# ruanyyyyyyy/point-cloud-process

Hardware: AMD Instinct MI355X
Metric: correspondence-pairs/sec + ms/ICP-iter, 120k-pt KITTI pair (higher is better)
Workload: dtype f64; 1 GPU; point-to-point ICP iteration, 120000 x 120000 KITTI-shaped synthetic scan pair per GPU (BASELINE configs[1]); exact 1-NN via grid; nn=grid, pairs_per_gpu=1, points_src=120000, points_tgt=120000

## Files before the change

### point-cloud-process_amd/csrc/pcr_grid_search.hip

```cpp
#include <atomic>
#include <chrono>
#include <cmath>
#include <cstdlib>
#include <cstring>
#include "pcr_descent.h"
#include "pcr_icp_step.h"

constexpr unsigned int HARD_SCAN_T = 192;
constexpr int HARD_STACK = 160;
constexpr long long ID_NONE = 0x7fffffffffffffffll;
constexpr int H_NLIST = 32;
constexpr int H_CSTRIDE = 32;
__host__ __device__ static inline unsigned int hard_list_cap(long long nq) {
    const long long halves = (nq + 15) / 16;
    return (unsigned int)(((halves + H_NLIST - 1) / H_NLIST) * 16 + 64);
}

template <int G>
__device__ static inline void group_best(double& bd2, long long& bid, unsigned int& bpos) {
#pragma unroll
    for (int off = G / 2; off > 0; off >>= 1) {
        const double od2 = __shfl_xor(bd2, off, 64);
        const long long oid = __shfl_xor(bid, off, 64);
        const unsigned int opos = __shfl_xor(bpos, off, 64);
// ... 757 lines not shown
                win[k] = readlane_f64(bw[k], wl);
        }
    }
}

__global__ void __launch_bounds__(256)
grid_hard_kernel(pcr_grid_view gv, const work_item* __restrict__ list, const unsigned int* __restrict__ count_p, long long nq, double max_d2, int gated,
                 unsigned int* __restrict__ res_pos, double* __restrict__ res_d2, unsigned long long* __restrict__ dbg,
                 const pcr_icp_dev_state* __restrict__ st) {
    __shared__ hard_lds s_lds[4];
    if (st && st->stop) return;
    const int lane = threadIdx.x & 63, wave = threadIdx.x >> 6;
    hard_lds* L = &s_lds[wave];
    unsigned int l_cnt = lane < H_NLIST ? count_p[H_CSTRIDE * lane] : 0u;
    unsigned int l_inc = l_cnt;
#pragma unroll
    for (int off = 1; off < H_NLIST; off <<= 1) {
        const unsigned int o = __shfl_up(l_inc, off, 64);
        if (lane >= off) l_inc += o;
    }
    const unsigned int count = __shfl(l_inc, H_NLIST - 1, 64);
    const unsigned int l_exc = l_inc - l_cnt;
    const unsigned int l_cap = hard_list_cap(nq);
    for (unsigned int w = blockIdx.x * 4 + wave; w < count; w += gridDim.x * 4) {
        const int hl = (int)__ffsll((long long)__ballot(lane < H_NLIST && l_exc <= w && w < l_exc + l_cnt)) - 1;
        const work_item it = list[(size_t)hl * l_cap + (w - __shfl(l_exc, hl, 64))];
        const unsigned long long h_t0 = dbg ? __builtin_amdgcn_s_memtime() : 0;
        unsigned int h_steps = 0, h_pts = 0;
        int s_level0 = 0;
        double bd2;
        long long bid;
        unsigned int bpos;
        hard_search(gv, L, lane, it.ax, it.ay, it.az, gated ? fmin(it.best_d2, max_d2) : it.best_d2, it.best_pos != POS_NONE, bd2, bid, bpos, h_steps,
                    h_pts, s_level0);
        if (lane == 0) {
            res_pos[it.qi] = bpos;
            if (res_d2) res_d2[it.qi] = bd2;
            if (dbg && w < 60000) {
                dbg[(1 << 17) + w * 4 + 0] = __builtin_amdgcn_s_memtime() - h_t0;
                dbg[(1 << 17) + w * 4 + 1] = ((unsigned long long)h_steps << 32);
                dbg[(1 << 17) + w * 4 + 2] = h_pts;
                dbg[(1 << 17) + w * 4 + 3] = (unsigned long long)(it.best_pos != POS_NONE) | ((unsigned long long)(s_level0 + 1) << 8);
            }
        }
    }
}

constexpr int ACC_SETS = 32;
constexpr double GATE_KAPPA = 1.25;
constexpr int PASS_GROUPS = 32;
constexpr int PASS_SYNC_STRIDE = 32;
constexpr int PASS_SYNC_WORDS = PASS_SYNC_STRIDE * (PASS_GROUPS + 1);
constexpr unsigned long long ITEM_NONE = ~0ull;
constexpr unsigned int POISON_HI = 0xfffffffeu;
__device__ static inline unsigned long long item_poison(unsigned int pass_id) { return ((unsigned long long)POISON_HI << 32) | pass_id; }
#ifndef PCR_PASS_SPIN_LIMIT
#define PCR_PASS_SPIN_LIMIT (1u << 21)
#endif
constexpr unsigned int PASS_SPIN_LIMIT = PCR_PASS_SPIN_LIMIT;
constexpr int Q_BITS = 22;
constexpr unsigned long long Q_MASK = (1ull << Q_BITS) - 1ull;
constexpr long long PASS_MAX_NQ = 1ll << 26;
struct pass_args {
    unsigned long long* items;
    unsigned long long* sync;
    unsigned int cap;
    unsigned long long* acc;
    wt_xyz* prev_xyz;
    unsigned long long* gate_lb;
    unsigned long long* gate_est;
    double scale, inv_scale;
    double lin, inv_lin;
    pcr_icp_dev_state* st;
    pcr_icp_loop_args la;
    unsigned int* tile_cost;
    unsigned int pass_id;
    unsigned long long* host_block;
    unsigned int notify;
    unsigned int* plog;
};
constexpr int PASS_LOG_WORDS = 3 * PCR_ICP_MAX_LOG + 8;
constexpr size_t HOST_LOG_OFF = (sizeof(pcr_icp_dev_state) + 63) & ~(size_t)63;
constexpr size_t HOST_FLAG_OFF = 8192 - 8;
static_assert(HOST_LOG_OFF + 4 * PASS_LOG_WORDS <= HOST_FLAG_OFF, "state + pass log + flag fit the landing block");
__host__ __device__ static inline unsigned int pass_item_cap(long long nq) {
    const long long tiles = (nq + WT_Q - 1) / WT_Q + 4;
    return (unsigned int)(((tiles + PASS_GROUPS - 1) / PASS_GROUPS) * (WT_Q + 1));
}

__device__ static inline long long to_fixed(double v, double scale) {
    constexpr double BIG = 6755399441055744.0;
    return __double_as_longlong(__builtin_fma(v, scale, BIG)) - __double_as_longlong(BIG);
}

__device__ static inline bool mom_is_linear(int k) { return k >= 1 && k <= 6; }
__device__ static inline void acc_fixed_add(unsigned long long* __restrict__ acc, unsigned int set, int lane, double mk, double scale, double lin) {
    if (lane < PCR_NMOM - 1 && mk != 0.0)
        atomicAdd(acc + (size_t)(set % ACC_SETS) * PCR_NMOM + lane, (unsigned long long)to_fixed(mk, mom_is_linear(lane) ? scale * lin : scale));
}

__device__ static inline void acc_fixed_add_ll(unsigned long long* __restrict__ acc, unsigned int set, int lane, long long v) {
    if (lane < PCR_NMOM - 1 && v != 0) atomicAdd(acc + (size_t)(set % ACC_SETS) * PCR_NMOM + lane, (unsigned long long)v);
}

__device__ static inline unsigned long long ld_dev(const unsigned long long* p) {
    return __hip_atomic_load(p, __ATOMIC_RELAXED, __HIP_MEMORY_SCOPE_AGENT);
}
__device__ static inline void st_dev(unsigned long long* p, unsigned long long v) {
    __hip_atomic_store(p, v, __ATOMIC_RELAXED, __HIP_MEMORY_SCOPE_AGENT);
}

constexpr int LAND_WORD = 18, LAND_ROOT = 24;
constexpr int LAND_PUB_SHIFT = 20, LAND_IN_SHIFT = 42;
constexpr unsigned long long LAND_TILE_MASK = (1ull << LAND_PUB_SHIFT) - 1ull;
constexpr unsigned long long TICKET_FIN = 1ull << 63;
static_assert(LAND_IN_SHIFT - LAND_PUB_SHIFT == Q_BITS && LAND_IN_SHIFT + Q_BITS == 64, "landed word: 20 + 22 + 22 bits");
__device__ __forceinline__ static bool land_complete(unsigned long long now, unsigned int g_tiles) {
    return (unsigned int)(now & LAND_TILE_MASK) == g_tiles && ((now >> LAND_PUB_SHIFT) & Q_MASK) == (now >> LAND_IN_SHIFT);
}
__device__ __forceinline__ static bool land_report_item(unsigned long long* sync, int lane, unsigned int qi, unsigned int n_waves, unsigned int n_groups) {
    asm volatile("s_waitcnt vmcnt(0)" ::: "memory");
    int fin = 0;
    if (lane == 0) {
        const unsigned int pg = (qi / WT_Q) % PASS_GROUPS;
        const unsigned long long now = __hip_atomic_fetch_add(sync + (size_t)PASS_SYNC_STRIDE * pg + LAND_WORD, 1ull << LAND_IN_SHIFT, __ATOMIC_RELAXED, __HIP_MEMORY_SCOPE_AGENT) +
                                       (1ull << LAND_IN_SHIFT);
        if (land_complete(now, n_waves / PASS_GROUPS + (pg < n_waves % PASS_GROUPS ? 1u : 0u)))
            fin = __hip_atomic_fetch_add(sync + (size_t)PASS_SYNC_STRIDE * PASS_GROUPS + LAND_ROOT, 1ull, __ATOMIC_RELAXED, __HIP_MEMORY_SCOPE_AGENT) == (unsigned long long)(n_groups - 1u) ? 1 : 0;
    }
    return __builtin_amdgcn_readfirstlane(fin) != 0;
}
__device__ __forceinline__ static int ticket_root(unsigned long long* root, unsigned long long tg_old, bool left_by_poison, bool failed, bool fin, unsigned int n_groups,
                                                  int& fin_seen) {
    const bool g_clean = ((tg_old >> 32) & 0xffffull) != 0 || left_by_poison;
    const bool g_failed = ((tg_old >> 48) & 0x7fffull) != 0 || failed;
    const bool g_fin = (tg_old & TICKET_FIN) != 0 || fin;
    const unsigned long long tr_old = __hip_atomic_fetch_add(root, 1ull | (g_clean ? 1ull << 32 : 0ull) | (g_failed ? 1ull << 48 : 0ull) | (g_fin ? TICKET_FIN : 0ull), __ATOMIC_RELAXED,
                                                             __HIP_MEMORY_SCOPE_AGENT);
    if ((unsigned int)tr_old != n_groups - 1u) return 0;
    fin_seen = ((tr_old & TICKET_FIN) != 0 || g_fin) ? 1 : 0;
    int last = ((unsigned int)((tr_old >> 32) & 0xffffull) + (g_clean ? 1u : 0u) == n_groups) ? 1 : 2;
    if (((tr_old >> 48) & 0x7fffull) != 0 || g_failed) last = 3;
    return last;
}

union pass_lds {
    wtile_lds t;
    hard_lds h;
    double xch[WT_Q * (PCR_NMOM - 1)];
    long long xll[WT_Q * (PCR_NMOM - 1)];
};

__device__ __forceinline__ static unsigned int pass_serve_item(const pcr_grid_view& gv, pass_lds* L, const int lane, const unsigned long long w, const double max_d2,
                                                       const pass_args& A, unsigned int* __restrict__ res_pos, unsigned long long* __restrict__ dbg,
                                                       const unsigned int dbg_slot, const unsigned long long t_start) {
    const unsigned int w_lo = (unsigned int)w, w_hi = (unsigned int)(w >> 32);
    const double ax = __hiloint2double(__builtin_amdgcn_readlane((int)w_hi, 0), __builtin_amdgcn_readlane((int)w_lo, 0));
    const double ay = __hiloint2double(__builtin_amdgcn_readlane((int)w_hi, 1), __builtin_amdgcn_readlane((int)w_lo, 1));
    const double az = __hiloint2double(__builtin_amdgcn_readlane((int)w_hi, 2), __builtin_amdgcn_readlane((int)w_lo, 2));
    const unsigned int qi = (unsigned int)__builtin_amdgcn_readlane((int)w_lo, 3);
    const float cand_b2 = __uint_as_float((unsigned int)__builtin_amdgcn_readlane((int)w_hi, 3));
    const unsigned long long h_t0 = dbg ? __builtin_amdgcn_s_memtime() : 0;
    unsigned int h_steps = 0, h_pts = 0;
    int s_level0 = 0;
    double bd2;
    long long bid;
    unsigned int bpos;
    const bool have_cand = cand_b2 < INFINITY;
    const bool wide = A.gate_est != nullptr && !have_cand;
    const double wide_d2 = max_d2 * (GATE_KAPPA * GATE_KAPPA);
    bool inside = false;
    double win[3];
    hard_search(gv, &L->h, lane, ax, ay, az, have_cand ? fmin((double)cand_b2, max_d2) : (wide ? wide_d2 : max_d2), have_cand, bd2, bid, bpos, h_steps, h_pts, s_level0, win);
    wave_sync();
    if (bpos != POS_NONE) {
        if (lane == 0) {
            pcr_pt b;
            b.x = win[0]; b.y = win[1]; b.z = win[2]; b.id = 0;
            double m[PCR_NMOM];
#pragma unroll
            for (int k = 0; k < PCR_NMOM; ++k) m[k] = 0.0;
            moments_add(m, gv.origin, ax, ay, az, b, max_d2, 1);
            inside = m[0] != 0.0;
            if (!wide || inside) A.prev_xyz[qi] = wt_xyz{b.x, b.y, b.z};
#pragma unroll
            for (int k = 0; k < PCR_NMOM - 1; ++k) L->xch[k] = m[k];
        }
// ... 208 lines not shown
    const unsigned int g = tile % PASS_GROUPS;
    const unsigned int g_tiles = n_waves / PASS_GROUPS + (g < n_waves % PASS_GROUPS ? 1u : 0u);
    unsigned long long* const g_q = A.sync + (size_t)PASS_SYNC_STRIDE * g;
    unsigned long long* const g_started = g_q + 16;
    unsigned long long* const g_ticket = g_q + 17;
    unsigned long long* const items = A.items + (size_t)g * A.cap * 4;
    if (lane == 0) __hip_atomic_fetch_add(g_started, 1ull, __ATOMIC_RELAXED, __HIP_MEMORY_SCOPE_AGENT);
    const unsigned int n_groups = n_waves < (unsigned int)PASS_GROUPS ? n_waves : (unsigned int)PASS_GROUPS;
    wt_state S;
    wtile_search(*gvp, &L->t, tile, lane, P, q, nq, x, 1, 1, max_d2, 1, pcap, res_pos, nullptr, dbg, use_prev ? A.prev_xyz : nullptr, S, inline_queue ? A.sync + 16 : nullptr,
                 (unsigned int)PASS_SYNC_STRIDE, n_groups, n_waves, use_prev ? A.gate_lb : nullptr, A.gate_est, A.pass_id);
    tile_record_cost(S, lane, A.tile_cost, tile);
    if (dbg) rt_tile = __builtin_amdgcn_s_memrealtime();
    tile_nb nb;
    tile_neighbour(gv.pts, S, P, lane, nb);
    bool all_started = false;
    if (inline_queue) {
        all_started = S.probe != 0;
        if (!all_started) {
            unsigned long long sv = 0;
            if (lane < (int)n_groups) sv = ld_dev(A.sync + (size_t)PASS_SYNC_STRIDE * lane + 16);
            const bool ok = lane < (int)n_groups && (unsigned int)sv == n_waves / PASS_GROUPS + ((unsigned int)lane < n_waves % PASS_GROUPS ? 1u : 0u);
            all_started = __ballot(ok) == (n_groups >= 64 ? ~0ull : (1ull << n_groups) - 1ull);
        }
    }
    const bool unres = S.open && lane < WT_Q;
    const unsigned long long um = __ballot(unres);
    unsigned int mine = 0;
    bool have_claim = false;
    unsigned long long own = 0;
    unsigned long long* const root = A.sync + (size_t)PASS_SYNC_STRIDE * PASS_GROUPS;
    {
        unsigned int tg;
        const unsigned long long slot_w = publish_reserve(A.sync, um, unres, lane, g, n_groups, tg);
        asm volatile("" :: "v"(slot_w) : "memory");
        if (lane == 0)
            own = __hip_atomic_fetch_add(g_q, (1ull << (2 * Q_BITS)) | (all_started ? 1ull << Q_BITS : 0ull), __ATOMIC_RELAXED, __HIP_MEMORY_SCOPE_AGENT);
        if (unres) publish_store<true>(A.items, A.cap, tg, slot_w, S, (unsigned int)S.qi);
    }
    tile_fold_moments(L, lane, S, P, nb, gv.origin, max_d2, A.prev_xyz, A.scale, A.lin, A.acc, tile);
    wave_sync();
    int fin = 0;
    unsigned long long rt_fin = 0;
    {
        {
            const unsigned int o_lo = (unsigned int)__builtin_amdgcn_readfirstlane((int)(unsigned int)own), o_hi = (unsigned int)__builtin_amdgcn_readfirstlane((int)(unsigned int)(own >> 32));
            own = ((unsigned long long)o_hi << 32) | o_lo;
        }
        if (all_started) {
            have_claim = true;
            mine = (unsigned int)((own >> Q_BITS) & Q_MASK);
        }
        const bool g_last_tile = (unsigned int)(own >> (2 * Q_BITS)) == g_tiles - 1u && inline_queue;
        unsigned long long rep = 0;
        if (inline_queue) {
            asm volatile("s_waitcnt vmcnt(0)" ::: "memory");
            const unsigned long long inc = lane == 0 ? (1ull | ((unsigned long long)__popcll(um) << LAND_PUB_SHIFT)) : 1ull;
            unsigned long long* const p = lane == 0 ? g_q + LAND_WORD : root + 8;
            if (lane == 0 || (lane == 1 && g_last_tile)) rep = __hip_atomic_fetch_add(p, inc, __ATOMIC_RELAXED, __HIP_MEMORY_SCOPE_AGENT) + inc;
        }
        const unsigned long long land_now = ((unsigned long long)(unsigned int)__builtin_amdgcn_readlane((int)(unsigned int)(rep >> 32), 0) << 32) | (unsigned int)__builtin_amdgcn_readlane((int)(unsigned int)rep, 0);
        const bool g_landed = inline_queue && land_complete(land_now, g_tiles);
        const bool psn = g_last_tile && (unsigned int)__builtin_amdgcn_readlane((int)(unsigned int)rep, 1) == n_groups;
        unsigned long long c_old = 0, qw = 0;
        if (g_landed && lane == 0) c_old = __hip_atomic_fetch_add(root + LAND_ROOT, 1ull, __ATOMIC_RELAXED, __HIP_MEMORY_SCOPE_AGENT);
        if (psn) {
            if (lane == 0) st_dev(root + 8, 0ull);
            if (lane < (int)n_groups) qw = ld_dev(A.sync + (size_t)PASS_SYNC_STRIDE * lane);
        }
        if (g_landed) fin = (unsigned int)__builtin_amdgcn_readfirstlane((int)(unsigned int)c_old) == n_groups - 1u ? 1 : 0;
        if (dbg && fin) rt_fin = __builtin_amdgcn_s_memrealtime();
        if (psn) {
            const unsigned int R_l = (unsigned int)(qw & Q_MASK);
            for (unsigned int gg = 0; gg < n_groups; ++gg) {
                const unsigned int R = (unsigned int)__builtin_amdgcn_readlane((int)R_l, (int)gg);
                const unsigned int gt = n_waves / PASS_GROUPS + (gg < n_waves % PASS_GROUPS ? 1u : 0u);
                unsigned long long* const base_g = A.items + (size_t)gg * A.cap * 4;
                for (unsigned int k = lane; k < gt; k += 64) st_dev(base_g + (size_t)(R + k) * 4 + 3, item_poison(A.pass_id));
            }
        }
    }
    if (dbg) rt_acc = __builtin_amdgcn_s_memrealtime();
    if (dbg && lane == 0) {
        atomicAdd(&dbg[blockIdx.x * 4 + 1], S.dbg_pairs);
        atomicAdd(&dbg[blockIdx.x * 4 + 2], (unsigned long long)S.dbg_passes);
        atomicAdd(&dbg[blockIdx.x * 4 + 3], (unsigned long long)__popcll(um));
        atomicMax(&dbg[blockIdx.x * 4 + 0], __builtin_amdgcn_s_memtime() - t_start);
    }
    if (!inline_queue) return;
    bool failed = false, left_by_poison = false;
    while (!fin) {
        if (!have_claim) {
            if (!all_started) {
                unsigned long long sv = 0;
                if (lane < (int)n_groups) sv = ld_dev(A.sync + (size_t)PASS_SYNC_STRIDE * lane + 16);
                const bool ok = lane < (int)n_groups && (unsigned int)sv == n_waves / PASS_GROUPS + ((unsigned int)lane < n_waves % PASS_GROUPS ? 1u : 0u);
                all_started = __ballot(ok) == (n_groups >= 64 ? ~0ull : (1ull << n_groups) - 1ull);
            }
            if (all_started) {
                unsigned long long old = 0;
                if (lane == 0) old = __hip_atomic_fetch_add(g_q, 1ull << Q_BITS, __ATOMIC_RELAXED, __HIP_MEMORY_SCOPE_AGENT);
                const unsigned int o_lo = (unsigned int)__builtin_amdgcn_readfirstlane((int)(unsigned int)old), o_hi = (unsigned int)__builtin_amdgcn_readfirstlane((int)(unsigned int)(old >> 32));
                old = ((unsigned long long)o_hi << 32) | o_lo;
                mine = (unsigned int)((old >> Q_BITS) & Q_MASK);
            } else {
                unsigned long long qw = 0;
                if (lane == 0) qw = ld_dev(g_q);
                const unsigned int q_lo = (unsigned int)__builtin_amdgcn_readfirstlane((int)(unsigned int)qw), q_hi = (unsigned int)__builtin_amdgcn_readfirstlane((int)(unsigned int)(qw >> 32));
                qw = ((unsigned long long)q_hi << 32) | q_lo;
                mine = (unsigned int)((qw >> Q_BITS) & Q_MASK);
                if (mine >= (unsigned int)(qw & Q_MASK)) break;
                int got = 0;
                if (lane == 0) {
                    unsigned long long expect = qw;
                    got = __hip_atomic_compare_exchange_strong(g_q, &expect, qw + (1ull << Q_BITS), __ATOMIC_RELAXED, __ATOMIC_RELAXED, __HIP_MEMORY_SCOPE_AGENT) ? 1 : 0;
                }
                if (!__builtin_amdgcn_readfirstlane(got)) { ++n_casfail; continue; }
            }
        }
        have_claim = false;
        unsigned long long* it = items + (size_t)mine * 4;
        unsigned long long w = ITEM_NONE;
        bool poisoned = false;
        for (unsigned int spins = 0;; ++spins) {
            if (lane < 4) w = ld_dev(it + lane);
            const unsigned int w3_lo = (unsigned int)__builtin_amdgcn_readlane((int)(unsigned int)w, 3), w3_hi = (unsigned int)__builtin_amdgcn_readlane((int)(unsigned int)(w >> 32), 3);
            poisoned = w3_hi == POISON_HI && w3_lo == A.pass_id;
            const unsigned long long mk = __ballot(lane < 4 && w != ITEM_NONE && !(lane == 3 && w3_hi == POISON_HI));
            if (poisoned || mk == 0xfull) break;
            if (spins >= PASS_SPIN_LIMIT) { failed = true; break; }
            ++n_polls;
            __builtin_amdgcn_s_sleep(16);
        }
        if (failed) break;
        if (poisoned) { left_by_poison = true; break; }
        if (lane < 4) st_dev(it + lane, ITEM_NONE);
        ++n_items;
        const unsigned int qi_served = pass_serve_item(gv, L, lane, w, max_d2, A, res_pos, dbg, g + PASS_GROUPS * mine, t_start);
        if (land_report_item(A.sync, lane, qi_served, n_waves, n_groups)) {
            fin = 2;
            if (dbg) rt_fin = __builtin_amdgcn_s_memrealtime();
        }
    }
    const unsigned long long rt_loop = dbg ? __builtin_amdgcn_s_memrealtime() : 0;
    int last = 0, fin_seen = 0;
    unsigned long long tg_old = 0;
    if (!fin) {
        asm volatile("s_waitcnt vmcnt(0)" ::: "memory");
        if (lane == 0)
            tg_old = __hip_atomic_fetch_add(g_ticket, 1ull | (left_by_poison ? 1ull << 32 : 0ull) | (failed ? 1ull << 48 : 0ull), __ATOMIC_RELAXED, __HIP_MEMORY_SCOPE_AGENT);
    }
    auto stamp_wave = [&]() {
        if (dbg && lane == 0) {
            unsigned long long* d = dbg + (1 << 19) + (size_t)(blockIdx.x * 4 + wave) * 8;
            d[0] = rt_start; d[1] = rt_tile; d[2] = rt_acc; d[3] = rt_loop; d[4] = n_items; d[5] = n_polls | ((unsigned long long)n_casfail << 32); d[6] = S.dbg_pairs | ((unsigned long long)S.dbg_passes << 40) | ((unsigned long long)__popcll(um) << 48); d[7] = __builtin_amdgcn_s_memrealtime();
        }
    };
    if (!fin) {
        if (lane == 0 && (unsigned int)tg_old == g_tiles - 1u) last = ticket_root(root, tg_old, left_by_poison, failed, false, n_groups, fin_seen);
        stamp_wave();
        last = __builtin_amdgcn_readfirstlane(last);
        if (!last) return;
        fin_seen = __builtin_amdgcn_readfirstlane(fin_seen);
    }
    if (last == 3 && dbg_arg && lane == 0) atomicAdd(&dbg_arg[(1 << 19) - 16], 1ull);
    if (last >= 2 && !fin_seen) {
        unsigned long long qw = 0;
        if (lane < (int)n_groups) qw = ld_dev(A.sync + (size_t)PASS_SYNC_STRIDE * lane);
        const unsigned int r_l = (unsigned int)(qw & Q_MASK);
        const unsigned int c_l = last == 3 ? 0u : (unsigned int)((qw >> Q_BITS) & Q_MASK);
        unsigned long long left = __ballot(lane < (int)n_groups && c_l < r_l);
        while (left) {
            const int gg = (int)__ffsll((long long)left) - 1;
            left &= left - 1;
            const unsigned int c0 = (unsigned int)__builtin_amdgcn_readlane((int)c_l, gg), r0 = (unsigned int)__builtin_amdgcn_readlane((int)r_l, gg);
            for (unsigned int i = c0; i < r0; ++i) {
                unsigned long long* it = A.items + ((size_t)gg * A.cap + i) * 4;
                unsigned long long w = ITEM_NONE;
                bool arrived = false;
                const unsigned int patience = last == 3 ? 64u : (PASS_SPIN_LIMIT < (1u << 21) ? (1u << 21) : PASS_SPIN_LIMIT);
                bool served_before = false;
                for (unsigned int spins = 0; spins < patience; ++spins) {
                    if (lane < 4) w = ld_dev(it + lane);
                    const unsigned int w3_hi = (unsigned int)__builtin_amdgcn_readlane((int)(unsigned int)(w >> 32), 3);
                    if (__ballot(lane < 4 && w != ITEM_NONE && !(lane == 3 && w3_hi == POISON_HI)) == 0xfull) { arrived = true; break; }
                    if (last == 3 && __ballot(lane < 4 && w == ITEM_NONE) == 0xfull) { served_before = true; break; }
                    __builtin_amdgcn_s_sleep(2);
                }
                if (served_before) continue;
                if (lane < 4) st_dev(it + lane, ITEM_NONE);
                if (!arrived) { if (lane == 0) st_dev(root + 16, 1ull); continue; }
                pass_serve_item(gv, L, lane, w, max_d2, A, res_pos, dbg, 59999u, t_start);
            }
        }
        asm volatile("s_waitcnt vmcnt(0)" ::: "memory");
    }
    auto clean_sync = [&]() {
        if (lane < (int)n_groups) {
            st_dev(A.sync + (size_t)PASS_SYNC_STRIDE * lane, 0ull);
            st_dev(A.sync + (size_t)PASS_SYNC_STRIDE * lane + 16, 0ull);
            st_dev(A.sync + (size_t)PASS_SYNC_STRIDE * lane + 17, 0ull);
        }
        if (lane == 0) st_dev(root, 0ull);
    };
    if (!fin) {
        clean_sync();
        if (fin_seen) return;
        if (lane < (int)n_groups) st_dev(A.sync + (size_t)PASS_SYNC_STRIDE * lane + LAND_WORD, 0ull);
        if (lane == 0) st_dev(root + LAND_ROOT, 0ull);
    }
    if (dbg_arg && lane == 0) atomicAdd(&dbg_arg[(1 << 19) - (fin ? 15 : 14)], 1ull);
    if (dbg && lane == 0) {
        dbg[(1 << 19) - 6] = fin ? (unsigned long long)fin : 3ull;
        dbg[(1 << 19) - 5] = fin ? rt_fin : __builtin_amdgcn_s_memrealtime();
    }
    if (fin) __builtin_amdgcn_s_setprio(3);
    pass_finish(gv, L, lane, A, root, dbg, [&]() {
        if (!fin) return;
        if (lane == 0) tg_old = __hip_atomic_fetch_add(g_ticket, 1ull | TICKET_FIN, __ATOMIC_RELAXED, __HIP_MEMORY_SCOPE_AGENT);
    });
    if (!fin) return;
    if (lane < (int)n_groups) st_dev(A.sync + (size_t)PASS_SYNC_STRIDE * lane + LAND_WORD, 0ull);
    if (lane == 0) st_dev(root + LAND_ROOT, 0ull);
    if (lane == 0 && (unsigned int)tg_old == g_tiles - 1u) last = ticket_root(root, tg_old, false, false, true, n_groups, fin_seen);
    stamp_wave();
    last = __builtin_amdgcn_readfirstlane(last);
    if (!last) return;
    if (last == 3 && dbg_arg && lane == 0) atomicAdd(&dbg_arg[(1 << 19) - 16], 1ull);
    clean_sync();
}

__global__ void __launch_bounds__(256) __attribute__((amdgpu_waves_per_eu(PCR_WT_WAVES, 8)))
grid_drain_kernel(pcr_grid_view gv, double max_d2, unsigned int* __restrict__ res_pos, unsigned long long* __restrict__ dbg, pass_args A) {
    __shared__ pass_lds s_lds[4];
    if (A.st->stop) return;
    const unsigned long long t_start = dbg ? __builtin_amdgcn_s_memtime() : 0;
    const unsigned long long t_rt_start = __builtin_amdgcn_s_memrealtime();
    const int lane = threadIdx.x & 63, wave = threadIdx.x >> 6;
    pass_lds* L = &s_lds[wave];
    const drain_part dp = drain_partition(A.sync, lane);
    const unsigned int total = dp.total;
    const unsigned int n_waves = gridDim.x * 4;
    if (dbg && blockIdx.x == 0 && threadIdx.x == 0) dbg[(1 << 19) - 8] = total;
    if (A.plog && blockIdx.x == 0 && threadIdx.x == 0 && A.pass_id < (unsigned int)PCR_ICP_MAX_LOG) {
        A.plog[PCR_ICP_MAX_LOG + A.pass_id] = (unsigned int)t_rt_start | 1u;
        A.plog[2 * PCR_ICP_MAX_LOG + A.pass_id] = total;
    }
    for (unsigned int w_i = blockIdx.x * 4 + wave; w_i < total; w_i += n_waves)
        pass_serve_item(gv, L, lane, drain_take(dp, A.items, A.cap, w_i, lane), max_d2, A, res_pos, dbg, w_i, t_start);
    asm volatile("s_waitcnt vmcnt(0)" ::: "memory");
    unsigned long long* const root = A.sync + (size_t)PASS_SYNC_STRIDE * PASS_GROUPS;
    const unsigned int wid = blockIdx.x * 4 + wave;
    const unsigned int n_groups = n_waves < (unsigned int)PASS_GROUPS ? n_waves : (unsigned int)PASS_GROUPS;
    const unsigned int g = wid % n_groups;
    const unsigned int g_size = n_waves / n_groups + (g < n_waves % n_groups ? 1u : 0u);
    unsigned long long* const g_ticket = A.sync + (size_t)PASS_SYNC_STRIDE * g + 17;
    int last = 0;
    if (lane == 0) {
        if (__hip_atomic_fetch_add(g_ticket, 1ull, __ATOMIC_RELAXED, __HIP_MEMORY_SCOPE_AGENT) == (unsigned long long)(g_size - 1u)) {
            st_dev(g_ticket, 0ull);
            if (__hip_atomic_fetch_add(root, 1ull, __ATOMIC_RELAXED, __HIP_MEMORY_SCOPE_AGENT) == (unsigned long long)(n_groups - 1u)) {
                st_dev(root, 0ull);
                last = 1;
            }
// ... 105 lines not shown
        }
    }
    __syncthreads();
    if (!s_last) return;
    if (threadIdx.x < H_NLIST) hard_count[H_CSTRIDE * threadIdx.x] = 0;
    __shared__ double s_red[8][32];
    const int k = threadIdx.x & 31, slice = threadIdx.x >> 5;
    double v = 0.0;
    if (k < PCR_NMOM) {
        for (int b0 = slice; b0 < (int)gridDim.x; b0 += 64) {
            double t[8];
#pragma unroll
            for (int u = 0; u < 8; ++u) {
                const int b = b0 + 8 * u;
                t[u] = b < (int)gridDim.x ? partials[(long long)b * PCR_NMOM + k] : 0.0;
            }
#pragma unroll
            for (int u = 0; u < 8; ++u) v += t[u];
        }
    }
    s_red[slice][k] = v;
    __syncthreads();
    __shared__ double s_m[PCR_NMOM];
    if (slice == 0 && k < PCR_NMOM) {
        const double tot = ((s_red[0][k] + s_red[1][k]) + (s_red[2][k] + s_red[3][k])) + ((s_red[4][k] + s_red[5][k]) + (s_red[6][k] + s_red[7][k]));
        if (out) out[k] = tot;
        s_m[k] = tot;
    }
    if (st) {
        __syncthreads();
        if (threadIdx.x == 0) pcr::icp_step(st, s_m, gv.origin, la, st->r_diff, st->t_diff);
    }
}

struct grid_scratch {
    pcr_dev_block res_pos, res_d2;
    pcr_dev_block hard_list;
    pcr_dev_block prev_xyz;
    pcr_dev_block acc, items, tile_cost;
    unsigned int* const hard_count;
    explicit grid_scratch(pcr_ctx* ctx)
        : res_pos(ctx), res_d2(ctx), hard_list(ctx), prev_xyz(ctx), acc(ctx), items(ctx), tile_cost(ctx), hard_count(ctx->d_counters + PCR_HARD_COUNTERS) {}
};

static int grid_scratch_alloc(grid_scratch* sc, int64_t nq, bool want_d2, bool want_hard) {
    int rc;
    if ((rc = sc->res_pos.alloc(sizeof(unsigned int) * nq))) return rc;
    if (want_d2 && (rc = sc->res_d2.alloc(sizeof(double) * nq))) return rc;
    if (want_hard && (rc = sc->hard_list.alloc(sizeof(work_item) * (size_t)H_NLIST * hard_list_cap(nq)))) return rc;
    return PCR_OK;
}

struct pass_layout {
    size_t sync_word, log_word, est_word, lb_word, zero_words;
    unsigned int cap;
    unsigned long long item_words;
};
static pass_layout pass_scratch_layout(long long nq, int n_pairs, bool with_log, bool with_bounds = false) {
    pass_layout l;
    l.sync_word = (size_t)n_pairs * ACC_SETS * PCR_NMOM;
    l.log_word = l.sync_word + PASS_SYNC_WORDS;
    l.est_word = l.log_word + (with_log ? PASS_LOG_WORDS / 2 : 0);
    l.lb_word = l.est_word + (with_bounds ? (size_t)nq : 0);
    l.zero_words = l.lb_word + (with_bounds ? (size_t)nq : 0);
    l.cap = pass_item_cap(nq);
    l.item_words = 4ull * PASS_GROUPS * l.cap;
    return l;
}

static int wtile_blocks(int64_t nq) { return (int)((nq + 4 * WT_Q - 1) / (4 * WT_Q)); }
static int queue_blocks(const pcr_ctx* ctx, long long want) { return (int)(want < 8ll * ctx->cu_count ? (want < 1 ? 1 : want) : 8ll * ctx->cu_count); }

static unsigned int wtile_point_cap(const pcr_ctx* ctx, int64_t nq) {
    const int nblocks = (int)((nq + 63) / 64);
    return (unsigned int)WT_PR * (nblocks > 8 * ctx->cu_count ? WT_ROUNDS_LARGE : WT_ROUNDS_SMALL);
}
constexpr unsigned int WT_BUSY_CAP = WT_PR * 48;
constexpr int WT_XCD_REMAP = 1;

static int grid_search_enqueue(pcr_ctx* ctx, const pcr_index* idx, pcr_pt* q, int64_t nq, hipStream_t stream, const pcr_xform* x, int write_back,
                               double max_d2, bool gated, bool mark, const grid_scratch* sc, const pcr_icp_dev_state* st, bool use_prev = false) {
    const int nblocks = (int)((nq + 63) / 64);
    pcr_xform xi;
    pcr_xform_from_T(nullptr, &xi);
    if (mark) pcr_prof_mark(ctx, 0);
    {
        if (ctx->d_debug) hipMemsetAsync(ctx->d_debug, 0, sizeof(unsigned long long) * ((1 << 16) + 8 * (size_t)nblocks), stream);
        hipLaunchKernelGGL(grid_wtile_kernel, dim3(wtile_blocks(nq)), dim3(256), 0, stream, (const pcr_grid_view*)idx->d_view, q, (long long)nq, x ? *x : xi,
                           (x || st) ? 1 : 0, write_back, max_d2, gated ? 1 : 0, WT_XCD_REMAP, wtile_point_cap(ctx, nq), sc->res_pos.as<unsigned int>(),
                           sc->res_d2.as<double>(), sc->hard_list.as<work_item>(), sc->hard_count, ctx->d_debug, st, (const wt_xyz*)(use_prev ? sc->prev_xyz.p : nullptr));
    }
    if (mark) pcr_prof_mark(ctx, 1);
    hipLaunchKernelGGL(grid_hard_kernel, dim3(queue_blocks(ctx, (nq + 3) / 4)), dim3(256), 0, stream, idx->view, (const work_item*)sc->hard_list.p,
                       (const unsigned int*)sc->hard_count, (long long)nq, max_d2, gated ? 1 : 0, sc->res_pos.as<unsigned int>(), sc->res_d2.as<double>(),
                       ctx->d_debug, st);
    PCR_HIP(ctx, hipGetLastError());
    return PCR_OK;
}

int pcr_grid_nn1(pcr_ctx* ctx, const pcr_index* idx, pcr_cloud* qc, const pcr_xform* x, double max_d2, int32_t* d_idx, double* d_d2) {
    const bool gated = (max_d2 > 0) && std::isfinite(max_d2);
    int rc = pcr_cloud_morton_sort(ctx, qc, idx->cell);
    if (rc) return rc;
    const int64_t nq = qc->n;
    grid_scratch sc(ctx);
    if ((rc = grid_scratch_alloc(&sc, nq, true, true)) || (rc = grid_search_enqueue(ctx, idx, qc->d, nq, ctx->stream, x, 0, max_d2, gated, true, &sc, nullptr)))
        return rc;
    const int grid = (int)((nq + 255) / 256);
    hipLaunchKernelGGL(grid_finalize_nn1_kernel, dim3(grid), dim3(256), 0, ctx->stream, idx->view, (const pcr_pt*)qc->d, (long long)nq,
                       (const unsigned int*)sc.res_pos.p, (const double*)sc.res_d2.p, max_d2, gated ? 1 : 0, d_idx, d_d2, sc.hard_count);
    PCR_HIP(ctx, hipGetLastError());
    return PCR_OK;
}

int pcr_grid_icp_pass(pcr_ctx* ctx, const pcr_index* idx, pcr_cloud* qc, const pcr_xform* x, double max_d2, int write_back,
                      double* d_moments) {
    const bool gated = (max_d2 > 0) && std::isfinite(max_d2);
    int rc = pcr_cloud_morton_sort(ctx, qc, idx->cell);
// ... 64 lines not shown
}

static std::atomic<int> g_loops_in_flight[64];
struct loop_guard {
    std::atomic<int>& n;
    explicit loop_guard(int device) : n(g_loops_in_flight[(unsigned int)device % 64u]) { n.fetch_add(1); }
    ~loop_guard() { n.fetch_sub(1); }
};

bool pcr_grid_pass_fused(const pcr_index* idx, int64_t nq, const pcr_icp_params* params, double* scale, double* inv_scale, double* lin) {
    double sc_f = 0, sc_i = 0, sc_lin = 1.0;
    const bool gated = (params->max_d2 > 0) && std::isfinite(params->max_d2);
    const bool fused = gated && nq <= PASS_MAX_NQ && getenv("PCR_ICP_NO_FUSED") == nullptr &&
                       pcr_pass_fixed_scale(idx->lo, idx->hi, nq, params->max_d2, &sc_f, &sc_i, &sc_lin);
    if (scale) *scale = sc_f;
    if (inv_scale) *inv_scale = sc_i;
    if (lin) *lin = sc_lin;
    return fused;
}

int pcr_grid_icp_loop(pcr_ctx* ctx, const pcr_index* idx, pcr_cloud* qc, const pcr_icp_params* params, const double T0[16],
                      pcr_icp_result* res) {
    const loop_guard in_flight(ctx->device);
    const auto h_t0 = std::chrono::steady_clock::now();
    auto h_us = [&](std::chrono::steady_clock::time_point a) { return std::chrono::duration_cast<std::chrono::nanoseconds>(std::chrono::steady_clock::now() - a).count() / 1e3; };
    for (double& v : ctx->pass_host_us) v = 0.0;
    const char* const wait_s = getenv("PCR_PASS_INLINE");
    const int wait_env = wait_s ? atoi(wait_s) : -1;
    const bool gated = (params->max_d2 > 0) && std::isfinite(params->max_d2);
    const int64_t nq = qc->n;
    int grid = (int)((nq + 1023) / 1024);
    if (grid > ctx->cu_count) grid = ctx->cu_count;
    double sc_f = 0, sc_i = 0, sc_lin = 1.0;
    const bool fused = pcr_grid_pass_fused(idx, nq, params, &sc_f, &sc_i, &sc_lin);
    int rc = pcr_cloud_morton_sort(ctx, qc, idx->cell, !fused);
    if (rc) return rc;
    grid_scratch sc(ctx);
    pcr_dev_block st_blk(ctx);
    if ((rc = grid_scratch_alloc(&sc, nq, false, !fused)) || (rc = sc.prev_xyz.alloc(24 * (size_t)nq))) return rc;
    const char* const lb_s = getenv("PCR_PASS_GATE_LB");
    const bool gate_bounds = !(lb_s && atoi(lb_s) == 0);
    const pass_layout pl = pass_scratch_layout(nq, 1, true, gate_bounds);
    pass_args pa{};
    if (fused) {
        if ((rc = sc.acc.alloc(8 * pl.zero_words)) || (rc = sc.tile_cost.alloc(sizeof(unsigned int) * 4 * (size_t)wtile_blocks(nq))) ||
            (rc = sc.items.alloc(8 * pl.item_words)))
            return rc;
        pa.cap = pl.cap;
        pa.items = sc.items.as<unsigned long long>();
        pa.tile_cost = sc.tile_cost.as<unsigned int>();
        pa.acc = sc.acc.as<unsigned long long>();
        pa.sync = pa.acc + pl.sync_word;
        pa.plog = (unsigned int*)(pa.acc + pl.log_word);
        pa.prev_xyz = sc.prev_xyz.as<wt_xyz>();
        if (gate_bounds) {
            pa.gate_est = pa.acc + pl.est_word;
            pa.gate_lb = pa.acc + pl.lb_word;
        }
        pa.scale = sc_f;
        pa.inv_scale = sc_i;
        pa.lin = sc_lin;
        pa.inv_lin = 1.0 / sc_lin;
    }
    if ((rc = pcr_ensure_scratch(ctx, sizeof(double) * PCR_NMOM * (size_t)grid)) || (rc = st_blk.alloc(sizeof(pcr_icp_dev_state)))) return rc;
    pcr_icp_dev_state* const d_st = st_blk.as<pcr_icp_dev_state>();
    static_assert(sizeof(pcr_icp_dev_state) <= 8192, "state must fit the pinned staging buffer");
    pcr_icp_dev_state* h_st = (pcr_icp_dev_state*)ctx->h_state;
    memset(h_st, 0, sizeof(*h_st));
    pcr::icp_state_from_T0(T0, h_st);
    const pcr_icp_loop_args la = pcr_icp_loop_args_from(params);
    volatile unsigned long long* const h_flag = (volatile unsigned long long*)((char*)ctx->h_state + HOST_FLAG_OFF);
    if (fused) {
        void* dp = nullptr;
        if (hipHostGetDevicePointer(&dp, ctx->h_state, 0) == hipSuccess) pa.host_block = (unsigned long long*)dp;
        *h_flag = 0ull;
        h_flag[-1] = 0ull;
    }
    hipError_t e = hipSuccess;
    ctx->pass_host_us[0] = h_us(h_t0);
    if (fused) {
        pass_T0 t0;
        for (int i = 0; i < 16; ++i) t0.v[i] = T0[i];
        const int ib = (int)((pl.item_words + 256 * 8 - 1) / (256 * 8));
        hipLaunchKernelGGL(pass_init_kernel, dim3(ib < 1 ? 1 : (ib > 1024 ? 1024 : ib)), dim3(256), 0, ctx->stream, pa.acc, (unsigned int)pl.zero_words,
                           pa.items, pl.item_words, d_st, t0, pa.plog,
                           pa.host_block ? pa.host_block + HOST_FLAG_OFF / 8 - 1 : (unsigned long long*)nullptr);
        e = hipGetLastError();
    } else e = hipMemcpyAsync(d_st, h_st, sizeof(*h_st), hipMemcpyHostToDevice, ctx->stream);
    pa.st = d_st;
    pa.la = la;
    pcr_xform xi;
    pcr_xform_from_T(nullptr, &xi);
    int enq = 0;
    const double prof_before = ctx->prof_ms[0] + ctx->prof_ms[1] + ctx->prof_ms[2] + ctx->prof_ms[3];
    int chunk = params->min_iter > 2 ? params->min_iter : 2;
    if (ctx->profile) chunk = 1;
    while (e == hipSuccess && rc == PCR_OK && enq < params->max_iter) {
        if (chunk > params->max_iter - enq) chunk = params->max_iter - enq;
        if (chunk > 64) chunk = 64;
        for (int c = 0; c < chunk && rc == PCR_OK; ++c) {
            const bool use_prev = enq + c > 0;
            const bool one_generation = (nq + WT_Q - 1) / WT_Q <= 16ll * ctx->cu_count;
            const int inline_queue = wait_env >= 0 ? wait_env : ((one_generation && !ctx->shared_device && in_flight.n.load(std::memory_order_relaxed) == 1) ? 1 : 0);
            if (fused) {
                if (ctx->profile) pcr_prof_mark(ctx, 0);
                if (ctx->d_debug) hipMemsetAsync(ctx->d_debug, 0, sizeof(unsigned long long) * (inline_queue ? ((1 << 16) + 8 * (size_t)((nq + 63) / 64)) : ((size_t)1 << 19)), ctx->stream);
// ... 216 lines not shown
```

Baseline: 3.630 billion correspondences/s.

## Replace per-item poison stores with shared release words for queue shutdown

When the last tile of the pass finishes, waves used to store a poison marker into every pending item slot of every group. Now a small array of release words, each covering several item indices, is written once per range, and waiting waves poll the matching release word in an extra lane alongside the item slot. The aim is to cut the number of global stores in the shutdown broadcast and speed up how quickly idle waves notice the pass is over. The cost is an extra load per poll, more scratch memory, and added debug-counter atomics in the kernel.

```diff
diff --git a/point-cloud-process_amd/csrc/pcr_grid_search.hip b/point-cloud-process_amd/csrc/pcr_grid_search.hip
--- a/point-cloud-process_amd/csrc/pcr_grid_search.hip
+++ b/point-cloud-process_amd/csrc/pcr_grid_search.hip
@@ -833,8 +833,12 @@
 constexpr int PASS_SYNC_STRIDE = 32;
 constexpr int PASS_SYNC_WORDS = PASS_SYNC_STRIDE * (PASS_GROUPS + 1);
 constexpr unsigned long long ITEM_NONE = ~0ull;
-constexpr unsigned int POISON_HI = 0xfffffffeu;
-__device__ static inline unsigned long long item_poison(unsigned int pass_id) { return ((unsigned long long)POISON_HI << 32) | pass_id; }
+#ifndef PCR_PASS_REL_SHARE
+#define PCR_PASS_REL_SHARE 8
+#endif
+constexpr unsigned int PASS_REL_SHARE = PCR_PASS_REL_SHARE;
+static_assert(PASS_REL_SHARE >= 1 && (PASS_REL_SHARE & (PASS_REL_SHARE - 1)) == 0, "release words: a power of two of indices per word");
+__host__ __device__ static inline unsigned int pass_release_words(unsigned int cap) { return cap / PASS_REL_SHARE + 2; }
 #ifndef PCR_PASS_SPIN_LIMIT
 #define PCR_PASS_SPIN_LIMIT (1u << 21)
 #endif
@@ -845,6 +849,7 @@
 struct pass_args {
     unsigned long long* items;
     unsigned long long* sync;
+    unsigned long long* release;
     unsigned int cap;
     unsigned long long* acc;
     wt_xyz* prev_xyz;
@@ -911,9 +916,9 @@
     }
     return __builtin_amdgcn_readfirstlane(fin) != 0;
 }
-__device__ __forceinline__ static int ticket_root(unsigned long long* root, unsigned long long tg_old, bool left_by_poison, bool failed, bool fin, unsigned int n_groups,
+__device__ __forceinline__ static int ticket_root(unsigned long long* root, unsigned long long tg_old, bool left_by_release, bool failed, bool fin, unsigned int n_groups,
                                                   int& fin_seen) {
-    const bool g_clean = ((tg_old >> 32) & 0xffffull) != 0 || left_by_poison;
+    const bool g_clean = ((tg_old >> 32) & 0xffffull) != 0 || left_by_release;
     const bool g_failed = ((tg_old >> 48) & 0x7fffull) != 0 || failed;
     const bool g_fin = (tg_old & TICKET_FIN) != 0 || fin;
     const unsigned long long tr_old = __hip_atomic_fetch_add(root, 1ull | (g_clean ? 1ull << 32 : 0ull) | (g_failed ? 1ull << 48 : 0ull) | (g_fin ? TICKET_FIN : 0ull), __ATOMIC_RELAXED,
@@ -1228,33 +1233,42 @@
             mine = (unsigned int)((own >> Q_BITS) & Q_MASK);
         }
         const bool g_last_tile = (unsigned int)(own >> (2 * Q_BITS)) == g_tiles - 1u && inline_queue;
-        unsigned long long rep = 0;
+        unsigned long long rep = 0, grp = 0;
         if (inline_queue) {
+            if (lane == 1 && g_last_tile) grp = __hip_atomic_fetch_add(root + 8, 1ull, __ATOMIC_RELAXED, __HIP_MEMORY_SCOPE_AGENT) + 1ull;
             asm volatile("s_waitcnt vmcnt(0)" ::: "memory");
-            const unsigned long long inc = lane == 0 ? (1ull | ((unsigned long long)__popcll(um) << LAND_PUB_SHIFT)) : 1ull;
-            unsigned long long* const p = lane == 0 ? g_q + LAND_WORD : root + 8;
-            if (lane == 0 || (lane == 1 && g_last_tile)) rep = __hip_atomic_fetch_add(p, inc, __ATOMIC_RELAXED, __HIP_MEMORY_SCOPE_AGENT) + inc;
-        }
-        const unsigned long long land_now = ((unsigned long long)(unsigned int)__builtin_amdgcn_readlane((int)(unsigned int)(rep >> 32), 0) << 32) | (unsigned int)__builtin_amdgcn_readlane((int)(unsigned int)rep, 0);
-        const bool g_landed = inline_queue && land_complete(land_now, g_tiles);
-        const bool psn = g_last_tile && (unsigned int)__builtin_amdgcn_readlane((int)(unsigned int)rep, 1) == n_groups;
+            const unsigned long long inc = 1ull | ((unsigned long long)__popcll(um) << LAND_PUB_SHIFT);
+            if (lane == 0) rep = __hip_atomic_fetch_add(g_q + LAND_WORD, inc, __ATOMIC_RELAXED, __HIP_MEMORY_SCOPE_AGENT) + inc;
+        }
+        const bool psn = g_last_tile && (unsigned int)__builtin_amdgcn_readlane((int)(unsigned int)grp, 1) == n_groups;
         unsigned long long c_old = 0, qw = 0;
-        if (g_landed && lane == 0) c_old = __hip_atomic_fetch_add(root + LAND_ROOT, 1ull, __ATOMIC_RELAXED, __HIP_MEMORY_SCOPE_AGENT);
         if (psn) {
             if (lane == 0) st_dev(root + 8, 0ull);
             if (lane < (int)n_groups) qw = ld_dev(A.sync + (size_t)PASS_SYNC_STRIDE * lane);
         }
+        const unsigned long long land_now = ((unsigned long long)(unsigned int)__builtin_amdgcn_readlane((int)(unsigned int)(rep >> 32), 0) << 32) | (unsigned int)__builtin_amdgcn_readlane((int)(unsigned int)rep, 0);
+        const bool g_landed = inline_queue && land_complete(land_now, g_tiles);
+        if (g_landed && lane == 0) c_old = __hip_atomic_fetch_add(root + LAND_ROOT, 1ull, __ATOMIC_RELAXED, __HIP_MEMORY_SCOPE_AGENT);
+        if (psn) {
+            const unsigned int R_l = (unsigned int)(qw & Q_MASK);
+            if (dbg && lane < (int)n_groups) atomicOr(&dbg[(1 << 19) - 10], 1ull << (R_l % PASS_REL_SHARE % 64u));
+            const unsigned int rel_w = pass_release_words(A.cap);
+            const unsigned int per = (n_waves / PASS_GROUPS) / PASS_REL_SHARE + 2u;
+            const unsigned int per_sh = 32u - (unsigned int)__builtin_clz(per - 1u), total = n_groups << per_sh;
+            const unsigned long long tag = (unsigned long long)(A.pass_id + 1u) << 32;
+            for (unsigned int i0 = 0; i0 < total; i0 += 64u) {
+                const unsigned int i = i0 + (unsigned int)lane;
+                const unsigned int gg = i < total ? i >> per_sh : n_groups - 1u, k = i & ((1u << per_sh) - 1u);
+                const unsigned int R = (unsigned int)__shfl((int)R_l, (int)gg, 64);
+                const unsigned int gt = n_waves / PASS_GROUPS + (gg < n_waves % PASS_GROUPS ? 1u : 0u);
+                const unsigned int wd = R / PASS_REL_SHARE + k;
+                if (i < total && wd <= (R + gt - 1u) / PASS_REL_SHARE) st_dev(A.release + (size_t)gg * rel_w + wd, tag | R);
+            }
+            if (dbg && lane == 0) dbg[(1 << 19) - 7] = __builtin_amdgcn_s_memrealtime();
+        }
         if (g_landed) fin = (unsigned int)__builtin_amdgcn_readfirstlane((int)(unsigned int)c_old) == n_groups - 1u ? 1 : 0;
         if (dbg && fin) rt_fin = __builtin_amdgcn_s_memrealtime();
-        if (psn) {
-            const unsigned int R_l = (unsigned int)(qw & Q_MASK);
-            for (unsigned int gg = 0; gg < n_groups; ++gg) {
-                const unsigned int R = (unsigned int)__builtin_amdgcn_readlane((int)R_l, (int)gg);
-                const unsigned int gt = n_waves / PASS_GROUPS + (gg < n_waves % PASS_GROUPS ? 1u : 0u);
-                unsigned long long* const base_g = A.items + (size_t)gg * A.cap * 4;
-                for (unsigned int k = lane; k < gt; k += 64) st_dev(base_g + (size_t)(R + k) * 4 + 3, item_poison(A.pass_id));
-            }
-        }
+        if (dbg && psn && lane == 0) dbg[(1 << 19) - 9] = fin ? 1ull : 0ull;
     }
     if (dbg) rt_acc = __builtin_amdgcn_s_memrealtime();
     if (dbg && lane == 0) {
@@ -1264,7 +1278,7 @@
         atomicMax(&dbg[blockIdx.x * 4 + 0], __builtin_amdgcn_s_memtime() - t_start);
     }
     if (!inline_queue) return;
-    bool failed = false, left_by_poison = false;
+    bool failed = false, left_by_release = false;
     while (!fin) {
         if (!have_claim) {
             if (!all_started) {
@@ -1296,20 +1310,21 @@
         }
         have_claim = false;
         unsigned long long* it = items + (size_t)mine * 4;
+        const unsigned long long* const poll_p = lane == 4 ? A.release + (size_t)g * pass_release_words(A.cap) + mine / PASS_REL_SHARE : it + lane;
         unsigned long long w = ITEM_NONE;
-        bool poisoned = false;
+        bool released = false;
         for (unsigned int spins = 0;; ++spins) {
-            if (lane < 4) w = ld_dev(it + lane);
-            const unsigned int w3_lo = (unsigned int)__builtin_amdgcn_readlane((int)(unsigned int)w, 3), w3_hi = (unsigned int)__builtin_amdgcn_readlane((int)(unsigned int)(w >> 32), 3);
-            poisoned = w3_hi == POISON_HI && w3_lo == A.pass_id;
-            const unsigned long long mk = __ballot(lane < 4 && w != ITEM_NONE && !(lane == 3 && w3_hi == POISON_HI));
-            if (poisoned || mk == 0xfull) break;
+            if (lane < 5) w = ld_dev(poll_p);
+            const unsigned int rw_lo = (unsigned int)__builtin_amdgcn_readlane((int)(unsigned int)w, 4), rw_hi = (unsigned int)__builtin_amdgcn_readlane((int)(unsigned int)(w >> 32), 4);
+            released = rw_hi == A.pass_id + 1u && mine >= rw_lo;
+            const unsigned long long mk = __ballot(lane < 4 && w != ITEM_NONE);
+            if (released || mk == 0xfull) break;
             if (spins >= PASS_SPIN_LIMIT) { failed = true; break; }
             ++n_polls;
             __builtin_amdgcn_s_sleep(16);
         }
         if (failed) break;
-        if (poisoned) { left_by_poison = true; break; }
+        if (released) { left_by_release = true; break; }
         if (lane < 4) st_dev(it + lane, ITEM_NONE);
         ++n_items;
         const unsigned int qi_served = pass_serve_item(gv, L, lane, w, max_d2, A, res_pos, dbg, g + PASS_GROUPS * mine, t_start);
@@ -1324,7 +1339,7 @@
     if (!fin) {
         asm volatile("s_waitcnt vmcnt(0)" ::: "memory");
         if (lane == 0)
-            tg_old = __hip_atomic_fetch_add(g_ticket, 1ull | (left_by_poison ? 1ull << 32 : 0ull) | (failed ? 1ull << 48 : 0ull), __ATOMIC_RELAXED, __HIP_MEMORY_SCOPE_AGENT);
+            tg_old = __hip_atomic_fetch_add(g_ticket, 1ull | (left_by_release ? 1ull << 32 : 0ull) | (failed ? 1ull << 48 : 0ull), __ATOMIC_RELAXED, __HIP_MEMORY_SCOPE_AGENT);
     }
     auto stamp_wave = [&]() {
         if (dbg && lane == 0) {
@@ -1333,7 +1348,7 @@
         }
     };
     if (!fin) {
-        if (lane == 0 && (unsigned int)tg_old == g_tiles - 1u) last = ticket_root(root, tg_old, left_by_poison, failed, false, n_groups, fin_seen);
+        if (lane == 0 && (unsigned int)tg_old == g_tiles - 1u) last = ticket_root(root, tg_old, left_by_release, failed, false, n_groups, fin_seen);
         stamp_wave();
         last = __builtin_amdgcn_readfirstlane(last);
         if (!last) return;
@@ -1358,8 +1373,7 @@
                 bool served_before = false;
                 for (unsigned int spins = 0; spins < patience; ++spins) {
                     if (lane < 4) w = ld_dev(it + lane);
-                    const unsigned int w3_hi = (unsigned int)__builtin_amdgcn_readlane((int)(unsigned int)(w >> 32), 3);
-                    if (__ballot(lane < 4 && w != ITEM_NONE && !(lane == 3 && w3_hi == POISON_HI)) == 0xfull) { arrived = true; break; }
+                    if (__ballot(lane < 4 && w != ITEM_NONE) == 0xfull) { arrived = true; break; }
                     if (last == 3 && __ballot(lane < 4 && w == ITEM_NONE) == 0xfull) { served_before = true; break; }
                     __builtin_amdgcn_s_sleep(2);
                 }
@@ -1386,6 +1400,7 @@
         if (lane == 0) st_dev(root + LAND_ROOT, 0ull);
     }
     if (dbg_arg && lane == 0) atomicAdd(&dbg_arg[(1 << 19) - (fin ? 15 : 14)], 1ull);
+    if (dbg_arg && lane == 0 && fin == 1) atomicAdd(&dbg_arg[(1 << 19) - 17], 1ull);
     if (dbg && lane == 0) {
         dbg[(1 << 19) - 6] = fin ? (unsigned long long)fin : 3ull;
         dbg[(1 << 19) - 5] = fin ? rt_fin : __builtin_amdgcn_s_memrealtime();
@@ -1597,7 +1612,7 @@
 }
 
 struct pass_layout {
-    size_t sync_word, log_word, est_word, lb_word, zero_words;
+    size_t sync_word, log_word, rel_word, est_word, lb_word, zero_words;
     unsigned int cap;
     unsigned long long item_words;
 };
@@ -1605,10 +1620,11 @@
     pass_layout l;
     l.sync_word = (size_t)n_pairs * ACC_SETS * PCR_NMOM;
     l.log_word = l.sync_word + PASS_SYNC_WORDS;
-    l.est_word = l.log_word + (with_log ? PASS_LOG_WORDS / 2 : 0);
+    l.cap = pass_item_cap(nq);
+    l.rel_word = l.log_word + (with_log ? PASS_LOG_WORDS / 2 : 0);
+    l.est_word = l.rel_word + (with_log ? (size_t)PASS_GROUPS * pass_release_words(l.cap) : 0);
     l.lb_word = l.est_word + (with_bounds ? (size_t)nq : 0);
     l.zero_words = l.lb_word + (with_bounds ? (size_t)nq : 0);
-    l.cap = pass_item_cap(nq);
     l.item_words = 4ull * PASS_GROUPS * l.cap;
     return l;
 }
@@ -1779,6 +1795,7 @@
         pa.acc = sc.acc.as<unsigned long long>();
         pa.sync = pa.acc + pl.sync_word;
         pa.plog = (unsigned int*)(pa.acc + pl.log_word);
+        pa.release = pa.acc + pl.rel_word;
         pa.prev_xyz = sc.prev_xyz.as<wt_xyz>();
         if (gate_bounds) {
             pa.gate_est = pa.acc + pl.est_word;
```

New measurement: 3.867 billion correspondences/s, median of 6. 6.5% higher.
